# Forrest-Z/my-lidar-graph-slam

Hardware: AMD Instinct MI355X
Metric: scans/sec + p50 scan-match ms, 1081-beam vs 1000×1000@5cm grid, 1/2/4/8 GPU (higher is better)
Workload: dtype f64

## Files before the change

### include/lgs_hip.h

```cpp
#ifndef LGS_HIP_H
#define LGS_HIP_H

#include <stddef.h>
#include <stdint.h>

#ifdef __cplusplus
extern "C" {
#endif

#define LGS_ABI_VERSION 2

#define LGS_OK               0
#define LGS_ERR_INVALID_ARG  1
#define LGS_ERR_HIP          2
#define LGS_ERR_NO_DEVICE    3
#define LGS_ERR_OOM          4
#define LGS_ERR_INTERNAL     5

typedef struct lgs_ctx  lgs_ctx;
typedef struct lgs_grid lgs_grid;
typedef struct lgs_scan lgs_scan;

typedef struct { double x, y, theta; } lgs_pose2d;

// ... 47 lines not shown

#define LGS_OPT_GUARD_EPS     1
#define LGS_OPT_FORCE_DENSE   2
#define LGS_OPT_INJECT_INDEX  3
#define LGS_OPT_GUARD_CAP     4
#define LGS_OPT_PROFILE       5
#define LGS_OPT_PROFILE_MASK  7
#define LGS_OPT_SPIN_SYNC     8
#define LGS_OPT_SKIP_MASK     10
#define LGS_OPT_SUPER_PRUNE   9
#define LGS_OPT_RAY_CHUNK_KEYS 13
#define LGS_OPT_LANES_MIN_BATCH 11
#define LGS_OPT_LINSOLVE_SPLIT 17
#define LGS_OPT_HANDOFF_SPIN_US 18
#define LGS_OPT_PEER_COPY     19
#define LGS_OPT_PRUNE_MIN_SUPER 21
#define LGS_OPT_COOP_TILES    22
#define LGS_OPT_SORT_BARRIER_US 23
#define LGS_OPT_FINE_STAGED   24
#define LGS_OPT_SMALL_WINDOW  25
#define LGS_OPT_POST_RECORDS  26
#define LGS_OPT_FUSED_PLANES  27
#define LGS_OPT_PRIORITY_TAIL 28
#define LGS_OPT_HV_FULL       29
#define LGS_OPT_SPLIT_CHUNKS  30
#define LGS_OPT_DEVICE_HITS   31
#define LGS_OPT_SEED_WIDE     32
#define LGS_OPT_ZERO_TILES    33
#define LGS_OPT_DEVICE_TIMING 34
#define LGS_OPT_LEAN_PROJECT  35
#define LGS_OPT_PGCG_GRID_NODES 36
#define LGS_OPT_FAST_ROWS     37
#define LGS_OPT_HV_INZERO     38
#define LGS_OPT_POISON_WS     15
int  lgs_ctx_set_option(lgs_ctx* ctx, int option, double value);

int  lgs_debug_item_buffer(lgs_ctx* ctx, int item, int which, void* out, size_t cap, size_t* bytes);

int  lgs_debug_libm(lgs_ctx* ctx, int op, const double* x, int n, double* out);

int  lgs_debug_keysort(lgs_ctx* ctx, const unsigned* keys, unsigned* out, long long n, int lo, int bits);

int  lgs_debug_copy_counters(const lgs_ctx* ctx, long long* direct, long long* staged);

int  lgs_debug_offset_checks(lgs_ctx* ctx, int reset, unsigned long long* out);

typedef struct {
    char name[32];
    int64_t launches;
    double total_ms;
    double algo_bytes;
    double dispatch_ms;
} lgs_kernel_stat;
int  lgs_ctx_kernel_stats(lgs_ctx* ctx, lgs_kernel_stat* out, int cap);
int  lgs_ctx_reset_stats(lgs_ctx* ctx);
int  lgs_ctx_match_counters(lgs_ctx* ctx, int64_t* out4);

int  lgs_grid_create(lgs_ctx* ctx, int w, int h, double min_x, double min_y,
                     double resolution, lgs_grid** out);
int  lgs_grid_wrap(lgs_ctx* ctx, double* device_cells, int w, int h, double min_x,
                   double min_y, double resolution, lgs_grid** out);
void lgs_grid_destroy(lgs_grid* grid);
int  lgs_grid_upload(lgs_ctx* ctx, lgs_grid* grid, const double* host_cells);
int  lgs_grid_upload_patches(lgs_ctx* ctx, lgs_grid* grid, const void* const* patches, int npx, int npy,
                             int patch_size, int cell_bytes, int value_offset);
int  lgs_grid_download(lgs_ctx* ctx, const lgs_grid* grid, double* host_cells);
// ... 449 lines not shown
```

### my-lidar-graph-slam_amd/csrc/k_rtcsm.hip

```cpp
#include "lgs_internal.hpp"
#include "loop_host.hpp"
#include "fast_cell.hpp"
#include "hv_zero.hpp"
#include "sq_cost_stage.hpp"
#include "ge_cost_device.hpp"

#include <algorithm>
#include <cfloat>
#include <cstring>
#include <map>
#include <mutex>
#include <thread>
#include <type_traits>

using namespace lgs;

namespace lgs {
void launch_precompute(lgs_ctx* ctx, const lgs_grid* in, int win, double* out, const PlaneGeom* planes);
void launch_precompute_jobs(lgs_ctx* ctx, const PrecompJob* d_jobs, int njobs, int maxW, int maxH, int win);
bool precompute_planes_ok(const lgs_grid* in, int win);
void precompute_tile_grid(int maxW, int maxH, int win, int njobs, int* gx, int* gy, int* rows);
}

namespace {
// ... 2571 lines not shown
        const int sg = seg_of(pref, nseg, b);
        const long long k = list[(size_t)sg * kSelSeg + (b - pref[sg])];
        double f;
        int pos;
        if constexpr (LR > 0)
            eval_block_t<LR, kFineDepth>(pl, grid, idx, zero, k, smem, sv, sk, f, pos, it % R);
        else
            eval_block(pl, grid, idx, zero, k, (int2*)smem, f, pos);
        if (threadIdx.x == 0) {
            fval[it] = f;
            fpos[it] = pos;
        }
        LGS_PROBE_MARK();
    }
    LGS_PROBE_PRINT("fine(seg_prefix, item0[, item1])");
}

__global__ __launch_bounds__(256) void k_compact(Items items)
{
    const MatchItem& it = items[blockIdx.x];
    extern __shared__ int pref[];
    __shared__ int ws[16];
    seg_prefix(it.segcnt, it.nseg, pref, ws);
    const int lane = threadIdx.x & 63, w = threadIdx.x >> 6;
    for (int sg = w; sg < it.nseg; sg += 4) {
        const int c = pref[sg + 1] - pref[sg];
        const int* __restrict__ src = it.list + (size_t)sg * kSelSeg;
        int* __restrict__ dst = it.dlist + pref[sg];
        for (int i = lane; i < c; i += 64) dst[i] = src[i];
    }
    if (threadIdx.x == 0) *it.nsel = pref[it.nseg];
}

constexpr int kFineLanesWaves = 1;
constexpr int kFineLanesMaxNv = 2048;
__global__ __launch_bounds__(64 * kFineLanesWaves) void k_fine_lanes(Items items, int n,
                                                                    const double* __restrict__ zero)
{
    __shared__ int ipref[kMaxBatchItems + 1];
    extern __shared__ int2 sidx[];
    if (threadIdx.x < 64) {
        const int j = threadIdx.x;
        const int c = (j < n) ? *items[j].nsel : 0;
        int incl = c;
        for (int off = 1; off < 64; off <<= 1) {
            const int t = __shfl_up(incl, off, 64);
            if (j >= off) incl += t;
        }
        if (j < n) ipref[j + 1] = incl;
        if (j == 0) ipref[0] = 0;
    }
    __syncthreads();
    const int total = ipref[n];
    const int lane = threadIdx.x & 63;
    for (int g = blockIdx.x; g < total; g += gridDim.x) {
        int lo = 0, hi = n - 1;
        while (lo < hi) {
            const int mid = (lo + hi + 1) >> 1;
            if (ipref[mid] <= g) lo = mid;
            else hi = mid - 1;
        }
        const int j = __builtin_amdgcn_readfirstlane(lo);
        const MatchItem& it = items[j];
        const RtcsmPlan& pl = it.pl;
        const int b = __builtin_amdgcn_readfirstlane(g - ipref[j]);
        const int k = it.dlist[b];
// ... 967 lines not shown
inline size_t align256(size_t b) { return (b + 255) & ~(size_t)255; }

struct BatchShape {
    int n = 0;
    int Tmax = 0, NvMax = 0, nsegMax = 0, nparts_max = 0;
    int P = 0, nsb2 = 0, chunks = 0, low_res = 0, cb = 0;
    bool pair = false;
    bool oct = false;
    int unit8 = 2;
    int nsby = 0;
    bool pruned = false;
    bool small = false;
    bool lr5 = false;
    bool fine_lanes = false;
    bool fine_staged = false;
    int frows = 1;
    int kernel_size = 0;
    bool sq = false;
    bool gx = false;
    WorkList wl{};
};

inline int item_nparts(const BatchShape& B, const RtcsmPlan& pl, bool pruned)
{
    return pruned ? B.chunks * pl.T : ((B.P + B.cb - 1) / B.cb) * pl.T;
}

inline bool uses_super(const lgs_ctx* ctx, int nv_max, int nsb2, bool dense)
{
    return !(dense || ctx->force_dense) && ctx->super_prune && nv_max <= kSeedMaxNv &&
           nsb2 <= 64 && nsb2 >= ctx->prune_min_super;
}

struct ItemLayout {
    size_t idx, cbase, cscore, cflag, list, segcnt, dlist, fval, fpos, part_c, part_k, sbound, poses7, cidx,
        terms, count, btab, atab, total;
};
ItemLayout item_layout(int Tmax, int NvMax, int P, int nsb2, int chunks, int cb, int frows, int Nmax)
{
    ItemLayout L{};
    size_t o = 0;
    auto take = [&](size_t bytes) {
        const size_t r = o;
        o += align256(std::max<size_t>(bytes, 16));
        return r;
    };
    const size_t K = (size_t)Tmax * P;
    const size_t nidx = (size_t)Tmax * std::max(NvMax, 1) + kPad;
    const size_t nseg = (K + kSelSeg - 1) / kSelSeg;
    const size_t nparts = std::max<size_t>((size_t)((P + cb - 1) / cb) * Tmax, (size_t)chunks * Tmax);
    L.idx = take(sizeof(int2) * nidx);
    L.cbase = take(sizeof(int) * 2 * nidx);
    L.cscore = take(sizeof(double) * K);
    L.cflag = take(K);
    L.list = take(sizeof(int) * nseg * kSelSeg);
    L.segcnt = take(sizeof(int) * nseg);
    L.dlist = take(sizeof(int) * K);
    L.fval = take(sizeof(double) * K * frows);
    L.fpos = take(sizeof(int) * K * frows);
    L.part_c = take(sizeof(double) * nparts);
    L.part_k = take(sizeof(long long) * nparts);
    L.sbound = take(sizeof(double) * (size_t)Tmax * std::max(nsb2, 1));
    L.poses7 = take(sizeof(double) * 21);
    L.cidx = take(sizeof(int4) * 7 * (size_t)Nmax);
    L.terms = take(sizeof(double) * 7 * (size_t)Nmax);
    L.count = take(128 + 24 * kSeedWide);
// ... 495 lines not shown
        const MatchItem& it = items[0];
        LGS_HIP_CHECK(hipMemcpyAsync(it.idx, opt.host_idx->data(), sizeof(int2) * opt.host_idx->size(),
                                     hipMemcpyHostToDevice, st));
        const size_t m = std::max<size_t>((size_t)it.pl.T * it.pl.Nv, kPad);
        hipLaunchKernelGGL(k_cinfo, dim3((unsigned)((m + 255) / 256)), dim3(256), 0, st, d_items);
        LGS_HIP_CHECK(hipGetLastError());
    } else {
        const bool lone = n < ctx->lanes_min_batch;
        const int rows = lone ? kProjRowsLone : kProjRows;
        dim3 g(std::max(1, (B.NvMax + 255) / 256), (B.Tmax + rows - 1) / rows, n);
        const int tok_ = ctx->timing_begin(K_PROJECT, items[0].lean ? 32.0 * B.NvMax * n : 24.0 * beams_T);
        if (ctx->skipped(K_PROJECT)) {
        } else if (items[0].lean)
            hipLaunchKernelGGL(k_beams, dim3(std::max(1, (B.NvMax + 255) / 256), 1, n), dim3(256), 0, st, d_items,
                               ctx->dts(tok_));
        else if (lone)
            hipLaunchKernelGGL(HIP_KERNEL_NAME(k_project<kProjRowsLone>), g, dim3(256), 0, st, d_items, ctx->guard_cap,
                               ctx->guard_eps, inject, ctx->dts(tok_));
        else
            hipLaunchKernelGGL(HIP_KERNEL_NAME(k_project<kProjRows>), g, dim3(256), 0, st, d_items, ctx->guard_cap,
                               ctx->guard_eps, inject, ctx->dts(tok_));
        ctx->timing_end(tok_);
        LGS_HIP_CHECK(hipGetLastError());
        if (opt.patches && !opt.patches->empty()) {
            int4* dp = (int4*)ctx->ensure(S_PATCH, sizeof(int4) * opt.patches->size());
            LGS_HIP_CHECK(hipMemcpyAsync(dp, opt.patches->data(), sizeof(int4) * opt.patches->size(),
                                         hipMemcpyHostToDevice, st));
            const int np = (int)opt.patches->size();
            hipLaunchKernelGGL(k_patch, dim3((np + 255) / 256), dim3(256), 0, st, d_items, dp, np);
            LGS_HIP_CHECK(hipGetLastError());
        }
    }
    const bool dense = opt.dense || ctx->force_dense;
    if (B.pruned) {
        {
            const int tok = ctx->timing_begin(K_SUPER, 8.0 * B.nsb2 * beams_T);
            const int oct_row_pad =
                std::max(kOctRowPad, kSupWaves * (64 / std::max(items[0].pl.nsbx, 1)) * std::max(LGS_OCT_PIPE5, LGS_OCT_PIPE9));
            const size_t lds = sizeof(int) * ((size_t)std::max(B.NvMax, 1) + (size_t)(B.oct ? oct_row_pad : kOctRowPad));
            dim3 g(B.chunks, B.Tmax, n);
            const bool packed = B.oct && oct_packed_ok(items);
            if (ctx->skipped(K_SUPER)) {
            } else if (B.oct && B.nsby <= 5 && packed)
                hipLaunchKernelGGL(HIP_KERNEL_NAME(k_super_oct<5, 2, 1>), g, dim3(64 * kSupWaves), lds, st, d_items, zero, ctx->dts(tok));
            else if (B.oct && packed)
                hipLaunchKernelGGL(HIP_KERNEL_NAME(k_super_oct<9, 3, 1>), g, dim3(64 * kSupWaves), lds, st, d_items, zero, ctx->dts(tok));
            else if (B.oct && B.nsby <= 5)
                hipLaunchKernelGGL(HIP_KERNEL_NAME(k_super_oct<5, 2, 0>), g, dim3(64 * kSupWaves), lds, st, d_items, zero, ctx->dts(tok));
            else if (B.oct)
                hipLaunchKernelGGL(HIP_KERNEL_NAME(k_super_oct<9, 3, 0>), g, dim3(64 * kSupWaves), lds, st, d_items, zero, ctx->dts(tok));
            else if (B.pair)
                hipLaunchKernelGGL(HIP_KERNEL_NAME(k_super<1>), g, dim3(64 * kSupWaves), lds, st, d_items, zero);
            else
                hipLaunchKernelGGL(HIP_KERNEL_NAME(k_super<0>), g, dim3(64 * kSupWaves), lds, st, d_items, zero);
            ctx->timing_end(tok);
            LGS_HIP_CHECK(hipGetLastError());
        }
        {
            const int tok = ctx->timing_begin(K_SEED, 8.0 * kSeedCands * (B.low_res * B.low_res + 16.0) * B.NvMax * n);
            const size_t lds = ((sizeof(int) * (size_t)std::max(B.NvMax, 1) + 15) & ~(size_t)15) +
                               sizeof(int2) * (size_t)std::max(B.NvMax, 1);
            const int nwide = std::min(ctx->seed_wide, kSeedWide);
            bool wide = nwide > kSeedCands && n >= ctx->lanes_min_batch;
            for (const auto& itm : items) wide = wide && itm.nparts <= kSeedWideMaxParts;
            if (!ctx->skipped(K_SEED) && wide) {
                hipLaunchKernelGGL(k_seed_members, dim3(nwide, n), dim3(kSeedMembersThreads),
                                   sizeof(int) * (size_t)std::max(B.NvMax, 1), st, d_items, ctx->dts(tok));
                hipLaunchKernelGGL(HIP_KERNEL_NAME(k_seed_super<2>), dim3(kSeedCands, n), dim3(LGS_SEED2_THREADS), lds, st,
                                   d_items, zero, ctx->dts(tok));
            } else if (!ctx->skipped(K_SEED))
                hipLaunchKernelGGL(HIP_KERNEL_NAME(k_seed_super<0>), dim3(kSeedCands, n), dim3(1024), lds, st,
                                   d_items, zero, ctx->dts(tok));
            else if (B.wl.cnt)
                LGS_HIP_CHECK(hipMemsetAsync(B.wl.cnt, 0, sizeof(int) * 16 * (size_t)n, st));
            ctx->timing_end(tok);
            LGS_HIP_CHECK(hipGetLastError());
        }
        const bool wl = n >= ctx->lanes_min_batch && B.wl.cnt && !ctx->skipped(K_COARSE);
        if (wl) {
            const int tk = ctx->timing_begin(K_COARSE_AUX, 8.0 * (double)B.Tmax * B.nsb2 * n);
            hipLaunchKernelGGL(k_keep, dim3(B.Tmax, n), dim3(64), 0, st, d_items, B.wl, ctx->dts(tk));
            ctx->timing_end(tk);
            LGS_HIP_CHECK(hipGetLastError());
        }
        const int tok = ctx->timing_begin(K_COARSE, 8.0 * beams_K);
        if (tok >= 0) ctx->pending[tok].coarse_evals = true;
        if (ctx->skipped(K_COARSE)) {
        } else if (wl) {
            hipLaunchKernelGGL(k_coarse_list_c, dim3(kListWaves), dim3(64), 0, st, d_items, B.wl, n, zero, ctx->dts(tok));
        } else {
            const size_t lds = ((sizeof(int) * (size_t)B.NvMax + 15) & ~(size_t)15) +
                               sizeof(double) * 128 * kRing * kRowWaves;
            hipLaunchKernelGGL(k_coarse_rows, dim3(B.Tmax, kSB, kRowSplit * n), dim3(64 * kRowWaves), lds, st,
                               d_items, zero);
        }
        ctx->timing_end(tok);
        LGS_HIP_CHECK(hipGetLastError());
        if (wl) {
            const int tk = ctx->timing_begin(K_COARSE_AUX, 0.0);
            hipLaunchKernelGGL(k_unsafe_list, dim3(std::min(kUnsafeGroups, n * B.Tmax)), dim3(64 * kLaneWaves), 0, st,
                               d_items, B.wl, n, zero, ctx->dts(tk));
            ctx->timing_end(tk);
            LGS_HIP_CHECK(hipGetLastError());
        }
    } else {
        {
            dim3 g((B.P + B.cb - 1) / B.cb, B.Tmax, n);
            const int tok = ctx->timing_begin(K_COARSE, 8.0 * beams_K);
            hipLaunchKernelGGL(k_coarse, g, dim3(B.cb), 0, st, d_items, zero);
            ctx->timing_end(tok);
            LGS_HIP_CHECK(hipGetLastError());
        }
        const int tok = ctx->timing_begin(K_SEED, 8.0 * B.low_res * B.low_res * (double)B.NvMax * n);
        if (B.lr5)
            hipLaunchKernelGGL(k_seed<5>, dim3(1, n), dim3(64 * 5), eval_t_smem<5>(B.NvMax), st, d_items, zero,
                               dense ? 1 : 0);
        else
            hipLaunchKernelGGL(k_seed<0>, dim3(1, n), dim3(64), sidx_bytes(B.NvMax), st, d_items, zero,
                               dense ? 1 : 0);
        ctx->timing_end(tok);
        LGS_HIP_CHECK(hipGetLastError());
    }
    {
        const int tok_ = ctx->timing_begin(K_SELECT, 10.0 * (double)B.Tmax * B.P * n);
        if (!ctx->skipped(K_SELECT)) {
            if (n >= ctx->lanes_min_batch)
                hipLaunchKernelGGL(HIP_KERNEL_NAME(k_select<256>), dim3((unsigned)B.nsegMax, n), dim3(256), 0, st,
                                   d_items, B.pruned ? 1 : 0, ctx->dts(tok_));
            else
                hipLaunchKernelGGL(HIP_KERNEL_NAME(k_select<kSelSeg>), dim3((unsigned)B.nsegMax, n), dim3(kSelSeg), 0,
                                   st, d_items, B.pruned ? 1 : 0, ctx->dts(tok_));
        }
        ctx->timing_end(tok_);
        LGS_HIP_CHECK(hipGetLastError());
    }
    if (B.fine_lanes) {
        hipLaunchKernelGGL(k_compact, dim3(n), dim3(256), pref_bytes(B.nsegMax), st, d_items);
        LGS_HIP_CHECK(hipGetLastError());
        const int tok_ = ctx->timing_begin(K_FINE, 0.0);
        if (ctx->skipped(K_FINE)) {
        } else if (B.fine_staged && ctx->fine_staged) {
            hipLaunchKernelGGL(k_fine_regs, dim3(4096), dim3(64), sizeof(unsigned) * (size_t)(B.NvMax + kFrPad), st,
                               d_items, n, zero, ctx->dts(tok_));
        } else {
            hipLaunchKernelGGL(k_fine_lanes, dim3(4096), dim3(64 * kFineLanesWaves),
                               sizeof(int2) * (size_t)(B.NvMax + 4 * kPipe), st, d_items, n, zero);
        }
        ctx->timing_end(tok_);
        LGS_HIP_CHECK(hipGetLastError());
    } else {
        const int tok_ = ctx->timing_begin(K_FINE, 0.0);
        dim3 g(fine_grid(n), n);
        if (ctx->skipped(K_FINE)) {
        } else if (B.lr5) {
            const size_t e = (sizeof(int2) * (size_t)((B.NvMax + 1) & ~1) + sizeof(double) * 2 * 5 * 65 + 15) &
                             ~size_t(15);
            hipLaunchKernelGGL(k_fine<5>, g, dim3(64), e + pref_bytes(B.nsegMax), st, d_items, zero, (unsigned)e);
        } else {
            const size_t e = (sidx_bytes(B.NvMax) + 15) & ~size_t(15);
            hipLaunchKernelGGL(k_fine<0>, g, dim3(64), e + pref_bytes(B.nsegMax), st, d_items, zero, (unsigned)e);
        }
        ctx->timing_end(tok_);
        LGS_HIP_CHECK(hipGetLastError());
    }
    {
        const int tok_ = ctx->timing_begin(K_REPLAY, 0.0);
        if (!ctx->skipped(K_REPLAY))
            hipLaunchKernelGGL(k_replay, dim3(n), dim3(64), pref_bytes(B.nsegMax), st, d_items, ctx->dts(tok_));
        ctx->timing_end(tok_);
        LGS_HIP_CHECK(hipGetLastError());
// ... 346 lines not shown
        it.nseedm = std::min(ctx->seed_wide, kSeedWide);
        it.inject = ctx->inject_index ? 1 : 0;
        it.geps = ctx->guard_eps;
        it.gcap = ctx->guard_cap;
        set_fast_rows(it, ctx->fast_rows);
    }
    const bool lean = lean_rows(ctx, B, items);
    for (auto& it : items) it.lean = lean ? 1 : 0;
    ctx->dbg.assign((size_t)n, lgs_ctx::DbgItem{});
    for (int j = 0; j < n; ++j) {
        const MatchItem& ij = items[j];
        const RtcsmPlan& q = ij.pl;
        const size_t nidx = (size_t)q.T * std::max(q.Nv, 1) + kPad;
        const void* b[8] = { ij.sbound, ij.part_c, ij.part_k, ij.Lp, ij.tedge, ij.cbase, ij.idx, ij.cscore };
        const size_t sz[8] = { sizeof(double) * (size_t)q.T * B.nsb2, sizeof(double) * (size_t)ij.nparts,
                               sizeof(long long) * (size_t)ij.nparts, 64 + sizeof(double) * kSeedCands,
                               sizeof(int) * (size_t)q.T, sizeof(int) * 2 * nidx,
                               sizeof(int2) * (size_t)q.T * q.Nv, sizeof(double) * (size_t)q.K };
        lgs_ctx::DbgItem& d = ctx->dbg[j];
        for (int k = 0; k < 8; ++k) {
            d.buf[k] = b[k];
            d.bytes[k] = sz[k];
        }
        d.buf[8] = ij.cmap;
        d.bytes[8] = ij.cmap ? plane_bytes(q) : 0;
        d.buf[9] = ij.super;
        d.bytes[9] = ij.super ? super_bytes(q) : 0;
        const PlaneSet* dps = B.small ? nullptr : &sets[set_of[j]];
        d.buf[10] = dps ? dps->hv_in : nullptr;
        d.bytes[10] = dps ? dps->hv_in_bytes : 0;
        d.buf[11] = dps ? dps->hv_out : nullptr;
        d.bytes[11] = dps ? dps->hv_out_bytes : 0;
        d.gen = ij.gen;
    }
    const size_t items_off = up.append(items.data(), items.size());
    up.flush();
    if (!B.small) launch_sets(ctx, p0, sets, sj, up);
    struct StreamRestore {
        lgs_ctx* c;
        hipStream_t s;
        ~StreamRestore() { c->stream = s; }
    } restore{ ctx, ctx->stream };
    if (!B.small && ctx->prio_tail && ctx->hi) {
        LGS_HIP_CHECK(hipEventRecord(ctx->split_ev[ctx->bank], ctx->stream));
        LGS_HIP_CHECK(hipStreamWaitEvent(ctx->hi, ctx->split_ev[ctx->bank], 0));
        ctx->stream = ctx->hi;
    }
    enqueue_items(ctx, B, up.at<MatchItem>(items_off), items, ScanOptions{});
    F.post = ctx->post_records;
    if (F.post) {
        static_assert(sizeof(RtcsmRecord) % 16 == 0, "k_post copies 16-byte words");
        F.flag = h_flag;
        F.post_gen = (unsigned)ctx->next_stamp();
        *(volatile unsigned*)h_flag = 0u;
        const int n16 = (int)(rec_bytes / 16);
        const int n2 = ctx->dts_dev ? (int)(kDtsBytes / 16) : 0;
        hipLaunchKernelGGL(k_post, dim3(1), dim3(std::min(kPostThreads, (std::max(n16, n2) + 63) / 64 * 64)), 0,
                           ctx->stream, (const uint4*)d_rec, (uint4*)h_rec, (int)(rec_bytes / 16), h_flag, F.post_gen,
                           (const uint4*)ctx->dts_dev, (uint4*)ctx->dts_host, n2);
        LGS_HIP_CHECK(hipGetLastError());
    } else {
        LGS_HIP_CHECK(hipMemcpyAsync(h_rec, d_rec, rec_bytes, hipMemcpyDeviceToHost, ctx->stream));
        if (ctx->dts_dev)
            LGS_HIP_CHECK(hipMemcpyAsync(const_cast<unsigned long long*>(ctx->dts_host), ctx->dts_dev, kDtsBytes,
                                         hipMemcpyDeviceToHost, ctx->stream));
    }
// ... 274 lines not shown
                        cpatch.push_back(make_int4(cells[0], cells[1], cells[2], cells[3]));
                    }
            }
            const int np = (int)(cpatch.size() / 2);
            int4* dp = (int4*)ctx->ensure(S_PATCH, sizeof(int4) * std::max<size_t>(cpatch.size(), 1));
            LGS_HIP_CHECK(hipMemcpyAsync(dp, cpatch.data(), sizeof(int4) * cpatch.size(), hipMemcpyHostToDevice,
                                         ctx->stream));
            if (np) hipLaunchKernelGGL(k_cost_patch, dim3((np + 255) / 256), dim3(256), 0, ctx->stream,
                                       items[j].cidx, dp, np);
            hipLaunchKernelGGL(KCOST(ks), dim3(7, 1), dim3(kCostThreads), cost_lds(items), ctx->stream, d_items + j,
                               ctx->guard_cap, ctx->guard_eps, 0, 1, DevTs{});
            LGS_HIP_CHECK(hipGetLastError());
            LGS_HIP_CHECK(hipMemcpyAsync(&h_rec[j], d_rec + j, sizeof(RtcsmRecord), hipMemcpyDeviceToHost,
                                         ctx->stream));
            ctx->sync();
            out[j].fixups = 1;
        }
        const double* c = h_rec[j].costs;
        out[j].normalized_cost = c[0] / (double)scans[j]->n;
        out[j].estimated_pose = move_backward(best[j], scans[j]->rel);
        const double dl = grid->res, da = 1e-2;
        const double g[3] = { 0.5 * (c[1] - c[2]) / dl, 0.5 * (c[3] - c[4]) / dl, 0.5 * (c[5] - c[6]) / da };
        for (int a = 0; a < 3; ++a)
            for (int b = 0; b < 3; ++b) out[j].covariance[3 * a + b] = g[a] * g[b];
        out[j].covariance[0] += 0.01;
        out[j].covariance[4] += 0.01;
        out[j].covariance[8] += 0.01;
    }
}
}

extern "C" int lgs_debug_item_buffer(lgs_ctx* ctx, int item, int which, void* out, size_t cap, size_t* bytes)
{
    if (!ctx || which < 0 || which >= 12 || item < 0) return LGS_ERR_INVALID_ARG;
    return guarded(ctx, [&] {
        LGS_REQUIRE((size_t)item < ctx->dbg.size(), "no such item in the last correlative batch");
        const lgs_ctx::DbgItem& d = ctx->dbg[(size_t)item];
        const size_t n = d.bytes[which];
        if (bytes) *bytes = n;
        if (!out || cap == 0) return;
        const size_t k = std::min(cap, n);
        LGS_HIP_CHECK(hipSetDevice(ctx->device));
        ctx->sync();
        LGS_HIP_CHECK(hipMemcpy(out, d.buf[which], k, hipMemcpyDeviceToHost));
        if (which == 4) {
            int* f = (int*)out;
            for (size_t i = 0; i < k / sizeof(int); ++i) f[i] = f[i] == d.gen ? 1 : 0;
        }
    });
}

extern "C" int lgs_rtcsm_optimize_pose(lgs_ctx* ctx, const lgs_grid* grid, const lgs_grid* coarse,
                                       const lgs_rtcsm_params* params,
                                       const lgs_cost_ge_params* cost, const lgs_scan* scan,
                                       lgs_pose2d initial, double nthr, lgs_rtcsm_summary* out)
{
    if (!ctx || !out || !grid || !coarse || !scan) return LGS_ERR_INVALID_ARG;
    return guarded(ctx, [&] {
        std::vector<PlaneSet> sets(1);
        sets[0].coarse = coarse;
        const int set0 = 0;
        lgs_scan* s = const_cast<lgs_scan*>(scan);
        run_matches(ctx, params, cost, &grid, &s, &initial, 1, nthr, sets, &set0, out);
    });
}

extern "C" int lgs_rtcsm_optimize_pose_batch(lgs_ctx* ctx, const lgs_grid* grid,
                                             const lgs_grid* coarse, const lgs_rtcsm_params* params,
                                             const lgs_cost_ge_params* cost,
                                             const lgs_scan* const* scans,
// ... 587 lines not shown
```

### my-lidar-graph-slam_amd/csrc/lgs_core.hip

```cpp
#include "lgs_internal.hpp"
#include "hv_zero.hpp"

#include <atomic>
#include <condition_variable>
#include <cstring>
#include <mutex>
#include <thread>

#include <pthread.h>

using namespace lgs;

void* lgs_ctx::ensure(int slot, size_t bytes)
{
    if (bytes == 0) bytes = 16;
    if (buf_bytes[slot] >= bytes) return buf[slot];
    if (buf[slot]) {
        LGS_HIP_CHECK(hipStreamSynchronize(stream));
        LGS_HIP_CHECK(hipFree(buf[slot]));
        buf[slot] = nullptr;
        buf_bytes[slot] = 0;
    }
    size_t want = bytes + bytes / 4;
    void* p = nullptr;
// ... 485 lines not shown
        if (!(value >= 1.0)) return LGS_ERR_INVALID_ARG;
        ctx->ray_chunk_keys = (long long)std::min(value, (double)(1LL << 30));
        return LGS_OK;
    case LGS_OPT_SKIP_MASK: ctx->skip_mask = (unsigned)value; return LGS_OK;
    case LGS_OPT_POISON_WS: ctx->poison_ws = value != 0.0; return LGS_OK;
    case LGS_OPT_PEER_COPY: ctx->peer_staged = value != 0.0; return LGS_OK;
    case LGS_OPT_PRUNE_MIN_SUPER: ctx->prune_min_super = (int)value; return LGS_OK;
    case LGS_OPT_COOP_TILES: ctx->coop_tiles = (long long)value; return LGS_OK;
    case LGS_OPT_FINE_STAGED: ctx->fine_staged = value != 0.0; return LGS_OK;
    case LGS_OPT_SMALL_WINDOW: ctx->small_window = value != 0.0; return LGS_OK;
    case LGS_OPT_POST_RECORDS: ctx->post_records = value != 0.0; return LGS_OK;
    case LGS_OPT_FUSED_PLANES: ctx->fused_planes = value != 0.0; return LGS_OK;
    case LGS_OPT_PRIORITY_TAIL: ctx->prio_tail = value != 0.0; return LGS_OK;
    case LGS_OPT_DEVICE_TIMING: ctx->dev_timing = value != 0.0; return LGS_OK;
    case LGS_OPT_HV_FULL: ctx->hv_full = value != 0.0; return LGS_OK;
    case LGS_OPT_SPLIT_CHUNKS: ctx->split_chunks = value != 0.0; return LGS_OK;
    case LGS_OPT_DEVICE_HITS: ctx->device_hits = value != 0.0; return LGS_OK;
    case LGS_OPT_ZERO_TILES: ctx->zero_tiles = value != 0.0; return LGS_OK;
    case LGS_OPT_HV_INZERO: ctx->hv_inzero = value != 0.0; return LGS_OK;
    case LGS_OPT_LEAN_PROJECT: ctx->lean_project = value != 0.0; return LGS_OK;
    case LGS_OPT_FAST_ROWS: ctx->fast_rows = value != 0.0; return LGS_OK;
    case LGS_OPT_PGCG_GRID_NODES:
        if (!(value >= 0.0)) return LGS_ERR_INVALID_ARG;
        ctx->pg_grid_nodes = (int)std::min(value, 2147483647.0);
        return LGS_OK;
    case LGS_OPT_LOOP_SEARCH_MIN_PAIRS:
        if (!(value >= 0.0)) return LGS_ERR_INVALID_ARG;
        ctx->loop_min_pairs = (long long)std::min(value, 9.0e18);
        return LGS_OK;
    case LGS_OPT_LOOP_SEARCH_GROUP:
        if (!(value >= 0.0)) return LGS_ERR_INVALID_ARG;
        ctx->loop_group = (int)std::min(value, 134217728.0);
        return LGS_OK;
    case LGS_OPT_SEED_WIDE:
        if (!(value >= 0.0 && value <= 16.0)) return LGS_ERR_INVALID_ARG;
        ctx->seed_wide = (int)value;
        return LGS_OK;
    case LGS_OPT_SORT_BARRIER_US:
        if (value < 0) return LGS_ERR_INVALID_ARG;
        ctx->sort_barrier_us = (long long)value;
        return LGS_OK;
    case LGS_OPT_LINSOLVE_SPLIT: ctx->linsolve_split = value != 0.0; return LGS_OK;
    case LGS_OPT_HANDOFF_SPIN_US:
        if (value < 0.0) return LGS_ERR_INVALID_ARG;
        ctx->handoff_spin_us = (long long)value;
        return LGS_OK;
    case LGS_OPT_GUARD_CAP:
        ctx->guard_cap = (int)value;
        if (ctx->guard_cap < 0) ctx->guard_cap = 0;
        if (ctx->guard_cap > kGuardInline) ctx->guard_cap = kGuardInline;
        return LGS_OK;
    default: ctx->last_error = "unknown option"; return LGS_ERR_INVALID_ARG;
    }
}

__global__ void k_fill(double* __restrict__ d, size_t n, double v)
{
    size_t i = (size_t)blockIdx.x * blockDim.x + threadIdx.x;
    size_t stride = (size_t)gridDim.x * blockDim.x;
    for (; i < n; i += stride) d[i] = v;
}

extern "C" int lgs_grid_create(lgs_ctx* ctx, int w, int h, double min_x, double min_y,
                               double res, lgs_grid** out)
{
    if (!ctx || !out) return LGS_ERR_INVALID_ARG;
// ... 1009 lines not shown
```

### my-lidar-graph-slam_amd/csrc/lgs_internal.hpp

```cpp
#pragma once

#include <hip/hip_runtime.h>

#include <climits>
#include <cmath>
#include <cstdint>
#include <cstring>
#include <functional>
#include <stdexcept>
#include <string>
#include <type_traits>
#include <memory>
#include <map>
#include <mutex>
#include <atomic>
#include <condition_variable>
#include <utility>
#include <vector>

#include "lgs_hip.h"
#include "lgs_error.hpp"
#include "pose_host.hpp"

namespace lgs {
// ... 190 lines not shown
constexpr int kDtsSlots = 32;
constexpr unsigned long long kDtsMask = (1ull << 40) - 1ull;
struct DevTs {
    unsigned long long* w;
    unsigned long long tag;
};
__device__ __forceinline__ void dts_begin(const DevTs& d)
{
    if (d.w && threadIdx.x == 0 && threadIdx.y == 0) {
        const unsigned b = blockIdx.x + gridDim.x * (blockIdx.y + gridDim.y * blockIdx.z);
        if (b < (unsigned)kDtsSub) {
            const unsigned long long t = __builtin_amdgcn_s_memrealtime() & kDtsMask;
            __hip_atomic_fetch_max(d.w + 2 * b, d.tag | (kDtsMask - t), __ATOMIC_RELAXED, __HIP_MEMORY_SCOPE_AGENT);
        }
    }
}
__device__ __forceinline__ void dts_end(const DevTs& d)
{
    if (d.w && threadIdx.x == 0 && threadIdx.y == 0) {
        const unsigned b = blockIdx.x + gridDim.x * (blockIdx.y + gridDim.y * blockIdx.z);
        const unsigned nwg = gridDim.x * gridDim.y * gridDim.z;
        if (b + (unsigned)kDtsSub >= nwg || b % (unsigned)kDtsEvery == 0u) {
            const unsigned long long t = __builtin_amdgcn_s_memrealtime() & kDtsMask;
            const unsigned sub = (b + b / (unsigned)kDtsEvery) & (unsigned)(kDtsSub - 1);
            __hip_atomic_fetch_max(d.w + 2 * sub + 1, d.tag | t, __ATOMIC_RELAXED, __HIP_MEMORY_SCOPE_AGENT);
        }
    }
}
struct DtsScope {
    const DevTs d;
    __device__ explicit DtsScope(const DevTs& x) : d(x) { dts_begin(d); }
    __device__ ~DtsScope() { dts_end(d); }
};
}

struct lgs_ctx {
    int device = 0;
    hipStream_t stream = nullptr;
    std::string last_error;
    double guard_eps = 1e-9;
    bool force_dense = false;
    bool inject_index = false;
    int guard_cap = lgs::kGuardInline;
    bool super_prune = true;
    bool linsolve_split = true;
    long long handoff_spin_us = 200000;
#ifndef LGS_FINE_STAGED_DEFAULT
#define LGS_FINE_STAGED_DEFAULT 1
#endif
    bool fine_staged = LGS_FINE_STAGED_DEFAULT;
    long long coop_tiles = -1;
    long long sort_barrier_us = 50000;
    long long handoff_fallbacks = 0;
    bool peer_staged = false;
    int prune_min_super = 1;
    bool small_window = true;
    bool fused_planes = true;
    int seed_wide = 12;
    bool lean_project = true;
    bool fast_rows = true;
    bool zero_tiles = true;
    bool device_hits = true;
    bool split_chunks = false;
    bool hv_inzero = true;
    bool hv_full = false;
    bool prio_tail = false;
    hipStream_t hi = nullptr;
    hipEvent_t split_ev[2] = {};
    bool post_records = true;
    long long copies_direct = 0, copies_staged = 0;
    int lanes_min_batch = 2;
    long long ray_chunk_keys = 1LL << 28;
    int next_stamp();
    unsigned skip_mask = 0;
    bool skipped(int kernel) const { return (skip_mask >> kernel) & 1u; }
    bool poison_ws = false;
    struct DbgItem {
        const void* buf[12];
        size_t bytes[12];
        int gen;
    };
    std::vector<DbgItem> dbg;
    int generation = 0;
    void* buf[lgs::S_NUM_SLOTS] = {};
    size_t buf_bytes[lgs::S_NUM_SLOTS] = {};
    void* pinned = nullptr;
    size_t pinned_bytes = 0;
    void* pinned_up = nullptr;
    size_t pinned_up_bytes = 0;
    void* pinned_up_b = nullptr;
    size_t pinned_up_b_bytes = 0;
    bool up_busy[2] = { false, false };
    void* pinned_rec[2] = {};
    size_t pinned_rec_bytes[2] = {};
    int bank = 0;
    size_t tedge_zeroed[2] = {};
    int* tedge_buffer(size_t n);
    int* small_counters(size_t n);
    int banked(int slot) const
    {
        if (!bank) return slot;
        switch (slot) {
        case lgs::S_BATCH_WS: return lgs::S_BATCH_WS_B;
        case lgs::S_RECORDS: return lgs::S_RECORDS_B;
        case lgs::S_UPLOAD: return lgs::S_UPLOAD_B;
        case lgs::S_DECIM: return lgs::S_DECIM_B;
        case lgs::S_SUPER: return lgs::S_SUPER_B;
        case lgs::S_NEGFLAG: return lgs::S_NEGFLAG_B;
        case lgs::S_TEDGE: return lgs::S_TEDGE_B;
        case lgs::S_ZTILE: return lgs::S_ZTILE_B;
        default: return slot;
        }
    }
// ... 412 lines not shown
```

### my-lidar-graph-slam_amd/lgs_amd/abi.py

```python
from __future__ import annotations

import ctypes as C
import os
from collections import namedtuple
from typing import Optional, Sequence

import numpy as np

_HERE = os.path.dirname(os.path.abspath(__file__))
LIB_PATH = os.path.join(_HERE, "liblgs_hip.so")

LGS_OK = 0
LGS_OPT_GUARD_EPS = 1
LGS_OPT_FORCE_DENSE = 2
LGS_OPT_INJECT_INDEX = 3
LGS_OPT_GUARD_CAP = 4
LGS_OPT_PROFILE = 5
LGS_OPT_PROFILE_MASK = 7
LGS_OPT_SPIN_SYNC = 8
LGS_OPT_SUPER_PRUNE = 9
LGS_OPT_LANES_MIN_BATCH = 11
LGS_OPT_RAY_CHUNK_KEYS = 13
LGS_OPT_POISON_WS = 15
LGS_OPT_SKIP_MASK = 10
LGS_OPT_LINSOLVE_SPLIT = 17
LGS_OPT_HANDOFF_SPIN_US = 18
LGS_OPT_PEER_COPY = 19
LGS_OPT_PRUNE_MIN_SUPER = 21
LGS_OPT_COOP_TILES = 22
LGS_OPT_SORT_BARRIER_US = 23
LGS_OPT_FINE_STAGED = 24
LGS_OPT_SMALL_WINDOW = 25
LGS_OPT_POST_RECORDS = 26
LGS_OPT_FUSED_PLANES = 27
LGS_OPT_PRIORITY_TAIL = 28
LGS_OPT_HV_FULL = 29
LGS_OPT_SPLIT_CHUNKS = 30
LGS_OPT_DEVICE_HITS = 31
LGS_OPT_SEED_WIDE = 32
LGS_OPT_ZERO_TILES = 33
LGS_OPT_DEVICE_TIMING = 34
LGS_OPT_LEAN_PROJECT = 35
LGS_OPT_PGCG_GRID_NODES = 36
LGS_OPT_FAST_ROWS = 37
LGS_OPT_HV_INZERO = 38
KERNEL_IDS = ["k_project", "k_coarse", "k_seed", "k_select", "k_fine", "k_replay", "k_cost", "k_precompute",
              "k_linsolve", "k_ray_emit", "k_ray_apply", "k_super", "k_super_planes", "k_bb_score",
              "k_bb_expand", "k_coarse_aux", "k_match_small", "k_gs_score",
              "k_cost_sq", "k_cost_gx"]
MORE_KERNEL_IDS = ["k_loop_search"]
LGS_OPT_LOOP_SEARCH_MIN_PAIRS = 39
LGS_OPT_LOOP_SEARCH_GROUP = 40


class Pose2D(C.Structure):
    _fields_ = [("x", C.c_double), ("y", C.c_double), ("theta", C.c_double)]

    def tuple(self):
        return (self.x, self.y, self.theta)


class ScanHost(C.Structure):
    _fields_ = [
        ("ranges", C.POINTER(C.c_double)),
        ("angles", C.POINTER(C.c_double)),
        ("n", C.c_int),
        ("rel_sensor_pose", Pose2D),
        ("min_range", C.c_double),
        ("max_range", C.c_double),
    ]


class RtcsmParams(C.Structure):
    _fields_ = [
        ("low_resolution", C.c_int),
        ("range_x", C.c_double),
        ("range_y", C.c_double),
        ("range_theta", C.c_double),
        ("scan_range_max", C.c_double),
    ]


class CostGEParams(C.Structure):
    _fields_ = [
        ("usable_range_min", C.c_double),
# ... 1030 lines not shown
        v = [C.c_longlong() for _ in range(5)]
        self.check(self.lib.lgs_pg_lm_stats(self.h, *[C.byref(x) for x in v]), "pg_lm_stats")
        return dict(zip(("optimizes", "steps", "pose_uploads", "pose_downloads", "incidence_builds"),
                        [x.value for x in v]))

    def map(self, res: float, patch_size: int, ncx: int, ncy: int, center=(0.0, 0.0)) -> "Map":
        h = _P()
        self.check(self.lib.lgs_map_create(self.h, res, patch_size, ncx, ncy, center[0], center[1],
                                           C.byref(h)), "map_create")
        return Map(self, h)

    def construct_maps(self, maps, ranges, scans, poses, bp: "BuilderParams"):
        nm, n = len(maps), len(scans)
        mh = (_P * nm)(*[m.h for m in maps])
        lo = (C.c_int * nm)(*[int(a) for a, _ in ranges])
        hi = (C.c_int * nm)(*[int(b) for _, b in ranges])
        arr = (_P * n)(*[s.h for s in scans])
        ps = (Pose2D * n)(*[Pose2D(*p) for p in poses])
        self.check(self.lib.lgs_maps_construct_from_scans(self.h, mh, lo, hi, nm, arr, ps, n, C.byref(bp)),
                   "maps_construct_from_scans")

    def construct_global_map(self, res: float, patch_size: int, scans, poses, bp: "BuilderParams") -> "Map":
        n = len(scans)
        arr = (_P * n)(*[s.h for s in scans])
        ps = (Pose2D * n)(*[Pose2D(*p) for p in poses])
        h = _P()
        self.check(self.lib.lgs_map_construct_global(self.h, res, patch_size, arr, ps, n, C.byref(bp), C.byref(h)),
                   "map_construct_global")
        return Map(self, h)

    DEBUG_BUFFERS = {"sbound": (0, np.float64), "part_c": (1, np.float64), "part_k": (2, np.int64),
                     "L": (3, np.float64), "tedge": (4, np.int32), "cbase": (5, np.int32), "idx": (6, np.int32),
                     "cscore": (7, np.float64), "planes": (8, np.float64), "super": (9, np.float16),
                     "hv_inmask": (10, np.uint64), "hv_outmask": (11, np.uint64)}

    def debug_buffer(self, name: str, item: int = 0) -> np.ndarray:
        which, dt = self.DEBUG_BUFFERS[name]
        n = C.c_size_t()
        self.check(self.lib.lgs_debug_item_buffer(self.h, item, which, None, 0, C.byref(n)), "debug_item_buffer")
        out = np.zeros(n.value // np.dtype(dt).itemsize, dtype=dt)
        self.check(self.lib.lgs_debug_item_buffer(self.h, item, which, out.ctypes.data_as(_P), out.nbytes,
                                                  C.byref(n)),
                   "debug_item_buffer")
        return out

    def debug_libm(self, op: int, x) -> np.ndarray:
        x = np.ascontiguousarray(x, dtype=np.float64)
        out = np.zeros((len(x), 2) if op == 0 else len(x), dtype=np.float64)
        self.check(self.lib.lgs_debug_libm(self.h, op, x.ctypes.data_as(_P), len(x), out.ctypes.data_as(_P)),
                   "debug_libm")
        return out

    def copy_counters(self) -> dict:
        a, b = C.c_longlong(), C.c_longlong()
        self.check(self.lib.lgs_debug_copy_counters(self.h, C.byref(a), C.byref(b)), "debug_copy_counters")
        return {"direct": a.value, "staged": b.value}

    def offset_checks(self, reset: bool = True) -> dict:
        out = (C.c_ulonglong * 4)()
        self.check(self.lib.lgs_debug_offset_checks(self.h, 1 if reset else 0, out), "debug_offset_checks")
        return {"checked": out[0], "violations": out[1], "first": out[2], "first_base": out[3]}

    def debug_keysort(self, keys, lo: int, bits: int) -> np.ndarray:
        k = np.ascontiguousarray(keys, dtype=np.uint32)
        out = np.zeros_like(k)
        self.check(self.lib.lgs_debug_keysort(self.h, k.ctypes.data_as(_P), out.ctypes.data_as(_P), len(k), lo, bits),
                   "debug_keysort")
# ... 250 lines not shown
```

Baseline: 105,600.

## Select candidates from surviving-superblock worklist into LDS bitmap, fusing compaction

Adds a k_select_list kernel that walks only the worklist of surviving superblocks, tests each cell's coarse score against the threshold and bound, and sets bits in a shared-memory bitmap. It then scans the bitmap to write the segmented list and, when fine lanes are used, the dense list and count directly. This skips the separate k_compact launch. It is meant to avoid scanning every translation times position candidate in the select kernel. It is on by default when a worklist exists and the problem size is under a cap. It uses one 1024-thread block per item, which may limit parallelism and relies on atomics in LDS.

New measurement: 107,400, median of 6. 1.7% higher.

```diff
diff --git a/include/lgs_hip.h b/include/lgs_hip.h
--- a/include/lgs_hip.h
+++ b/include/lgs_hip.h
@@ -103,6 +103,7 @@
 #define LGS_OPT_PGCG_GRID_NODES 36
 #define LGS_OPT_FAST_ROWS     37
 #define LGS_OPT_HV_INZERO     38
+#define LGS_OPT_SELECT_LIST   41
 #define LGS_OPT_POISON_WS     15
 int  lgs_ctx_set_option(lgs_ctx* ctx, int option, double value);
 
diff --git a/my-lidar-graph-slam_amd/csrc/k_rtcsm.hip b/my-lidar-graph-slam_amd/csrc/k_rtcsm.hip
--- a/my-lidar-graph-slam_amd/csrc/k_rtcsm.hip
+++ b/my-lidar-graph-slam_amd/csrc/k_rtcsm.hip
@@ -2627,6 +2627,105 @@
     if (threadIdx.x == 0) *it.nsel = pref[it.nseg];
 }
 
+constexpr long long kSelListMaxK = 524288;
+constexpr int kSelListThreads = 1024;
+constexpr int kSelListU = 8;
+__global__ __launch_bounds__(kSelListThreads) void k_select_list(Items items, WorkList W, int dense, DevTs dts)
+{
+    const DtsScopeAll dts_scope(dts);
+    extern __shared__ unsigned long long s_bm[];
+    constexpr int kT = kSelListThreads, kW = kT / 64, kU = kSelListU, kRow = kT / 16;
+    const int j = blockIdx.x;
+    const MatchItem& it = items[j];
+    const RtcsmPlan& pl = it.pl;
+    const int tid = threadIdx.x, lane = tid & 63, wid = tid >> 6;
+    const int nwords = it.nseg * (kSelSeg / 64);
+    const int* __restrict__ sbl = W.sbl + (size_t)j * W.region;
+    const int cnt = min(W.cnt[16 * j], W.region);
+    int ent[kU];
+#pragma unroll
+    for (int u = 0; u < kU; ++u) {
+        const int e = (tid >> 4) + kRow * u;
+        ent[u] = e < cnt ? sbl[e] : -1;
+    }
+    for (int w = tid; w < nwords; w += kT) s_bm[w] = 0ull;
+    __syncthreads();
+    {
+        const double* __restrict__ cscore = it.cscore;
+        const uint8_t* __restrict__ cflag = it.cflag;
+        const double L = *it.Lp, thr = pl.thr;
+        const int nsbx = max(pl.nsbx, 1), m = tid & 15;
+        unsigned* bm32 = (unsigned*)s_bm;
+        for (int e0 = tid >> 4; e0 < cnt; e0 += kRow * kU) {
+            int k[kU];
+            double c[kU];
+            uint8_t fl[kU];
+#pragma unroll
+            for (int u = 0; u < kU; ++u) {
+                const int t = ent[u] >> 6, sb = ent[u] & 63;
+                const int jx = kSB * (sb % nsbx) + (m & 3), jy = kSB * (sb / nsbx) + (m >> 2);
+                const bool active = ent[u] >= 0 && t < pl.T && jx < pl.ncx && jy < pl.ncy;
+                k[u] = active ? t * pl.P + jx * pl.ncy + jy : -1;
+            }
+#pragma unroll
+            for (int u = 0; u < kU; ++u) {
+                c[u] = k[u] >= 0 ? cscore[k[u]] : 0.0;
+                fl[u] = k[u] >= 0 ? cflag[k[u]] : 0;
+            }
+#pragma unroll
+            for (int u = 0; u < kU; ++u) {
+                const int e = e0 + kRow * (kU + u);
+                ent[u] = e < cnt ? sbl[e] : -1;
+            }
+#pragma unroll
+            for (int u = 0; u < kU; ++u)
+                if (k[u] >= 0 && (c[u] > thr) && (fl[u] || c[u] >= L)) atomicOr(bm32 + (k[u] >> 5), 1u << (k[u] & 31));
+        }
+    }
+    __syncthreads();
+    int* __restrict__ list = it.list;
+    int* __restrict__ dlist = it.dlist;
+    int run = 0;
+    for (int w0 = 0; w0 < nwords; w0 += kT) {
+        const int w = w0 + tid;
+        unsigned long long v = w < nwords ? s_bm[w] : 0ull;
+        const int c = __popcll(v);
+        int incl = c;
+#pragma unroll
+        for (int off = 1; off < 64; off <<= 1) {
+            const int u = __shfl_up(incl, off, 64);
+            if (lane >= off) incl += u;
+        }
+        const int excl = incl - c;
+        const int seg0 = __shfl(excl, lane & ~15, 64);
+        const int segn = __shfl(incl, lane | 15, 64) - seg0;
+        if ((lane & 15) == 0 && w < nwords) it.segcnt[w >> 4] = segn;
+        int base = 0;
+        if (dense) {
+            static_assert(kW * sizeof(int) <= (kSelSeg / 64) * sizeof(unsigned long long), "totals fit one segment");
+            __syncthreads();
+            int* wt = (int*)(s_bm + w0);
+            if (lane == 63) wt[wid] = incl;
+            __syncthreads();
+            base = run;
+#pragma unroll
+            for (int q = 0; q < kW; ++q) {
+                const int tq = wt[q];
+                if (q < wid) base += tq;
+                run += tq;
+            }
+        }
+        int r = 0;
+        for (; v; v &= v - 1ull, ++r) {
+            const int key = (w << 6) + __ffsll((long long)v) - 1;
+            list[(size_t)(w >> 4) * kSelSeg + (excl - seg0) + r] = key;
+            if (dense) dlist[base + excl + r] = key;
+        }
+    }
+    if (dense && tid == 0) *it.nsel = run;
+    __syncthreads();
+}
+
 constexpr int kFineLanesWaves = 1;
 constexpr int kFineLanesMaxNv = 2048;
 __global__ __launch_bounds__(64 * kFineLanesWaves) void k_fine_lanes(Items items, int n,
@@ -3660,6 +3759,11 @@
            nsb2 <= 64 && nsb2 >= ctx->prune_min_super;
 }
 
+inline bool select_list_fits(const lgs_ctx* ctx, const BatchShape& B)
+{
+    return B.wl.cnt && (long long)B.Tmax * B.P <= std::min(ctx->select_list, kSelListMaxK);
+}
+
 struct ItemLayout {
     size_t idx, cbase, cscore, cflag, list, segcnt, dlist, fval, fpos, part_c, part_k, sbound, poses7, cidx,
         terms, count, btab, atab, total;
@@ -4221,6 +4325,7 @@
         }
     }
     const bool dense = opt.dense || ctx->force_dense;
+    bool wl = false;
     if (B.pruned) {
         {
             const int tok = ctx->timing_begin(K_SUPER, 8.0 * B.nsb2 * beams_T);
@@ -4265,7 +4370,7 @@
             ctx->timing_end(tok);
             LGS_HIP_CHECK(hipGetLastError());
         }
-        const bool wl = n >= ctx->lanes_min_batch && B.wl.cnt && !ctx->skipped(K_COARSE);
+        wl = n >= ctx->lanes_min_batch && B.wl.cnt && !ctx->skipped(K_COARSE);
         if (wl) {
             const int tk = ctx->timing_begin(K_COARSE_AUX, 8.0 * (double)B.Tmax * B.nsb2 * n);
             hipLaunchKernelGGL(k_keep, dim3(B.Tmax, n), dim3(64), 0, st, d_items, B.wl, ctx->dts(tk));
@@ -4310,9 +4415,14 @@
         ctx->timing_end(tok);
         LGS_HIP_CHECK(hipGetLastError());
     }
+    const bool sel_list = wl && select_list_fits(ctx, B) && !ctx->skipped(K_SELECT);
     {
         const int tok_ = ctx->timing_begin(K_SELECT, 10.0 * (double)B.Tmax * B.P * n);
-        if (!ctx->skipped(K_SELECT)) {
+        if (ctx->skipped(K_SELECT)) {
+        } else if (sel_list) {
+            hipLaunchKernelGGL(k_select_list, dim3(n), dim3(kSelListThreads), sizeof(unsigned long long) * 16 * (size_t)B.nsegMax,
+                               st, d_items, B.wl, B.fine_lanes ? 1 : 0, ctx->dts(tok_));
+        } else {
             if (n >= ctx->lanes_min_batch)
                 hipLaunchKernelGGL(HIP_KERNEL_NAME(k_select<256>), dim3((unsigned)B.nsegMax, n), dim3(256), 0, st,
                                    d_items, B.pruned ? 1 : 0, ctx->dts(tok_));
@@ -4324,7 +4434,7 @@
         LGS_HIP_CHECK(hipGetLastError());
     }
     if (B.fine_lanes) {
-        hipLaunchKernelGGL(k_compact, dim3(n), dim3(256), pref_bytes(B.nsegMax), st, d_items);
+        if (!sel_list) hipLaunchKernelGGL(k_compact, dim3(n), dim3(256), pref_bytes(B.nsegMax), st, d_items);
         LGS_HIP_CHECK(hipGetLastError());
         const int tok_ = ctx->timing_begin(K_FINE, 0.0);
         if (ctx->skipped(K_FINE)) {
@@ -4737,6 +4847,18 @@
         d.buf[11] = dps ? dps->hv_out : nullptr;
         d.bytes[11] = dps ? dps->hv_out_bytes : 0;
         d.gen = ij.gen;
+        if (!B.small) {
+            d.list = ij.list;
+            d.segcnt = ij.segcnt;
+            d.nseg = ij.nseg;
+            if (B.fine_lanes) {
+                d.nsel = ij.nsel;
+                d.dlist = ij.dlist;
+                d.K = (size_t)q.K;
+            }
+            d.sel_list = n >= ctx->lanes_min_batch && !ctx->skipped(K_COARSE) && !ctx->skipped(K_SELECT) &&
+                         select_list_fits(ctx, B);
+        }
     }
     const size_t items_off = up.append(items.data(), items.size());
     up.flush();
@@ -5077,10 +5199,32 @@
 
 extern "C" int lgs_debug_item_buffer(lgs_ctx* ctx, int item, int which, void* out, size_t cap, size_t* bytes)
 {
-    if (!ctx || which < 0 || which >= 12 || item < 0) return LGS_ERR_INVALID_ARG;
+    if (!ctx || which < 0 || which >= 16 || item < 0) return LGS_ERR_INVALID_ARG;
     return guarded(ctx, [&] {
         LGS_REQUIRE((size_t)item < ctx->dbg.size(), "no such item in the last correlative batch");
         const lgs_ctx::DbgItem& d = ctx->dbg[(size_t)item];
+        if (which >= 12) {
+            const void* src[2] = { nullptr, nullptr };
+            size_t sz[2] = { 0, 0 };
+            const int sel = d.sel_list;
+            if (which == 12 && d.list) src[0] = d.list, sz[0] = sizeof(int) * (size_t)d.nseg * kSelSeg;
+            if (which == 13 && d.segcnt) src[0] = d.segcnt, sz[0] = sizeof(int) * (size_t)d.nseg;
+            if (which == 14 && d.nsel) src[0] = d.nsel, sz[0] = sizeof(int), src[1] = d.dlist, sz[1] = sizeof(int) * d.K;
+            if (which == 15) sz[0] = sizeof(int);
+            if (bytes) *bytes = sz[0] + sz[1];
+            if (!out || cap == 0) return;
+            LGS_HIP_CHECK(hipSetDevice(ctx->device));
+            ctx->sync();
+            size_t done = 0;
+            for (int i = 0; i < 2; ++i) {
+                const size_t k = std::min(cap - done, sz[i]);
+                if (!k) continue;
+                if (src[i]) LGS_HIP_CHECK(hipMemcpy((char*)out + done, src[i], k, hipMemcpyDeviceToHost));
+                else memcpy((char*)out + done, &sel, std::min(k, sizeof(int)));
+                done += k;
+            }
+            return;
+        }
         const size_t n = d.bytes[which];
         if (bytes) *bytes = n;
         if (!out || cap == 0) return;
diff --git a/my-lidar-graph-slam_amd/csrc/lgs_core.hip b/my-lidar-graph-slam_amd/csrc/lgs_core.hip
--- a/my-lidar-graph-slam_amd/csrc/lgs_core.hip
+++ b/my-lidar-graph-slam_amd/csrc/lgs_core.hip
@@ -541,6 +541,10 @@
         if (!(value >= 0.0)) return LGS_ERR_INVALID_ARG;
         ctx->loop_group = (int)std::min(value, 134217728.0);
         return LGS_OK;
+    case LGS_OPT_SELECT_LIST:
+        if (!(value >= 0.0)) return LGS_ERR_INVALID_ARG;
+        ctx->select_list = (long long)std::min(value, 9.0e18);
+        return LGS_OK;
     case LGS_OPT_SEED_WIDE:
         if (!(value >= 0.0 && value <= 16.0)) return LGS_ERR_INVALID_ARG;
         ctx->seed_wide = (int)value;
diff --git a/my-lidar-graph-slam_amd/csrc/lgs_internal.hpp b/my-lidar-graph-slam_amd/csrc/lgs_internal.hpp
--- a/my-lidar-graph-slam_amd/csrc/lgs_internal.hpp
+++ b/my-lidar-graph-slam_amd/csrc/lgs_internal.hpp
@@ -246,6 +246,19 @@
     __device__ explicit DtsScope(const DevTs& x) : d(x) { dts_begin(d); }
     __device__ ~DtsScope() { dts_end(d); }
 };
+struct DtsScopeAll {
+    const DevTs d;
+    __device__ explicit DtsScopeAll(const DevTs& x) : d(x) { dts_begin(d); }
+    __device__ ~DtsScopeAll()
+    {
+        if (d.w && threadIdx.x == 0 && threadIdx.y == 0) {
+            const unsigned b = blockIdx.x + gridDim.x * (blockIdx.y + gridDim.y * blockIdx.z);
+            const unsigned long long t = __builtin_amdgcn_s_memrealtime() & kDtsMask;
+            __hip_atomic_fetch_max(d.w + 2 * (b & (unsigned)(kDtsSub - 1)) + 1, d.tag | t, __ATOMIC_RELAXED,
+                                   __HIP_MEMORY_SCOPE_AGENT);
+        }
+    }
+};
 }
 
 struct lgs_ctx {
@@ -283,6 +296,7 @@
     hipEvent_t split_ev[2] = {};
     bool post_records = true;
     long long copies_direct = 0, copies_staged = 0;
+    long long select_list = 524288;
     int lanes_min_batch = 2;
     long long ray_chunk_keys = 1LL << 28;
     int next_stamp();
@@ -293,6 +307,9 @@
         const void* buf[12];
         size_t bytes[12];
         int gen;
+        const int *list, *segcnt, *nsel, *dlist;
+        int nseg, sel_list;
+        size_t K;
     };
     std::vector<DbgItem> dbg;
     int generation = 0;
diff --git a/my-lidar-graph-slam_amd/lgs_amd/abi.py b/my-lidar-graph-slam_amd/lgs_amd/abi.py
--- a/my-lidar-graph-slam_amd/lgs_amd/abi.py
+++ b/my-lidar-graph-slam_amd/lgs_amd/abi.py
@@ -51,6 +51,7 @@
 MORE_KERNEL_IDS = ["k_loop_search"]
 LGS_OPT_LOOP_SEARCH_MIN_PAIRS = 39
 LGS_OPT_LOOP_SEARCH_GROUP = 40
+LGS_OPT_SELECT_LIST = 41
 
 
 class Pose2D(C.Structure):
@@ -1147,7 +1148,9 @@
     DEBUG_BUFFERS = {"sbound": (0, np.float64), "part_c": (1, np.float64), "part_k": (2, np.int64),
                      "L": (3, np.float64), "tedge": (4, np.int32), "cbase": (5, np.int32), "idx": (6, np.int32),
                      "cscore": (7, np.float64), "planes": (8, np.float64), "super": (9, np.float16),
-                     "hv_inmask": (10, np.uint64), "hv_outmask": (11, np.uint64)}
+                     "hv_inmask": (10, np.uint64), "hv_outmask": (11, np.uint64),
+                     "sel_list": (12, np.int32), "sel_segcnt": (13, np.int32), "sel_dense": (14, np.int32),
+                     "sel_by_list": (15, np.int32)}
 
     def debug_buffer(self, name: str, item: int = 0) -> np.ndarray:
         which, dt = self.DEBUG_BUFFERS[name]
```
